# sndels/prosper

Measured on AMD Instinct MI355X. Metric: Mpaths/s, higher is better.
Workload: dtype f32; 1 GPU; S-cornell 1920x1080 8spp maxBounces 4; width=1920, height=1080, spp=8, max_bounces=4, triangles=38, bvh_nodes=7, parallelism=image stripes x1, pipeline=wavefront, 3 frames in flight (one launch chain each)

## Files before the change

include/prosper_pt/prosper_pt.h:

```cpp
#ifndef PROSPER_PT_H
#define PROSPER_PT_H

#include <stddef.h>
#include <stdint.h>

#include "shader_structs.h"

#ifdef __cplusplus
extern "C" {
#endif

#define PROSPER_PT_ABI_VERSION 4

enum
{
    PROSPER_PT_OK = 0,
    PROSPER_PT_ERR_INVALID_ARGUMENT = -1,
    PROSPER_PT_ERR_NO_DEVICE = -2,
    PROSPER_PT_ERR_HIP = -3,
    PROSPER_PT_ERR_NO_SCENE = -4,
    PROSPER_PT_ERR_SCENE = -5,
    PROSPER_PT_ERR_UNSUPPORTED = -6,
};

// ... 126 lines not shown
typedef struct prosper_pt_scene_stats
{
    uint64_t triangleCount;
    uint64_t nodeCount;
    uint32_t nodeBytes;
    uint32_t triangleBytes;
    uint32_t maxDepth;
    uint32_t variantFlags;
    uint64_t deviceBytes;
    double buildSeconds;
    double uploadSeconds;
    double bvhBuildSeconds;
    double textureSeconds;
    uint64_t alphaTriangleCount;
    uint64_t alphaBoundBytes;
} prosper_pt_scene_stats;
enum
{
    PROSPER_PT_VARIANT_LDS_SCENE = 1u << 0,
    PROSPER_PT_VARIANT_LDS_TABLES = 1u << 1,
    PROSPER_PT_VARIANT_BATCHED_TEXTURES = 1u << 2,
    PROSPER_PT_VARIANT_TEXTURE_PACKS = 1u << 3,
    PROSPER_PT_VARIANT_RAW_RECORDS = 1u << 4,
    PROSPER_PT_VARIANT_STACK_SHIFT = 8,
};

enum
{
    PROSPER_PT_RENDER_COUNT_WORK = 1u << 0,
    PROSPER_PT_RENDER_PIPELINED = 1u << 1,
};

typedef struct prosper_pt_debug_options
{
    uint32_t struct_size;
    int32_t batchedTextures;
    int32_t widePacks;
    int32_t alphaCellShift;
    uint32_t noTexturePacks;
    uint32_t noAlphaBounds;
    uint32_t noUploadRefit;
    uint32_t flatBvh;
    float sahTraversalCost;
    float boxPad;
    uint32_t leafSize;
    uint32_t buildThreads;
    uint32_t topEntries;
    int32_t nodeOrder;
    int32_t childOrder;
    uint32_t buildTiming;
    uint32_t segments;
    uint32_t segmentLength;
    uint32_t chains;
    uint32_t ldsStackEntries;
    uint32_t noLdsScene;
    uint32_t noLdsTables;
    uint32_t traceDeadPaths;
    int32_t bandedBatches;
    float rebuildCostRatio;
    uint32_t alwaysRebuild;
    uint32_t failNextUpdate;
    uint32_t poolVariant;
    uint32_t rawRecords;
    uint32_t tileOrder;
    uint32_t hipGraph;
    uint32_t pipelinedChains;
    uint32_t mergeLimit;
} prosper_pt_debug_options;

const char *prosper_pt_last_error(void);
uint32_t prosper_pt_abi_version(void);
uint32_t prosper_pt_has_experiments(void);
void prosper_pt_debug_options_default(prosper_pt_debug_options *out);
int prosper_pt_set_debug_options(prosper_pt_ctx *ctx, const prosper_pt_debug_options *options);
int prosper_pt_get_debug_options(prosper_pt_ctx *ctx, prosper_pt_debug_options *out);

int prosper_pt_create(const prosper_pt_device_desc *desc, prosper_pt_ctx **out_ctx);
void prosper_pt_destroy(prosper_pt_ctx *ctx);

int prosper_pt_upload_scene(prosper_pt_ctx *ctx, const prosper_pt_scene_view *scene);
int prosper_pt_update_lights(
    prosper_pt_ctx *ctx, const prosper_DirectionalLightParameters *directionalLight,
    const prosper_PointLightsBuffer *pointLights, const prosper_SpotLightsBuffer *spotLights);
int prosper_pt_update_transforms(prosper_pt_ctx *ctx, const prosper_ModelInstanceTransforms *transforms, uint32_t count);
enum
{
    PROSPER_PT_UPDATE_NOW = 1u << 0,
};
int prosper_pt_update_transforms_async(
    prosper_pt_ctx *ctx, const prosper_ModelInstanceTransforms *transforms, uint32_t count, uint32_t flags, void *stream);
// ... 228 lines not shown
```

prosper_amd/csrc/prosper_pt.cpp:

```cpp
#include "../../include/prosper_pt/prosper_pt.h"

#include <hip/hip_runtime.h>

#include <algorithm>
#include <chrono>
#include <future>
#include <memory>
#include <cmath>
#include <cstdlib>
#include <cstdio>
#include <cstring>
#include <exception>
#include <stdexcept>
#include <string>
#include <vector>

#include "bvh_build.hpp"
#include "pt_context.hpp"
#include "pt_geometry.hpp"
#include "pt_kernels.hpp"
#include "pt_materials.hpp"
#include "pt_pass_support.hpp"
#include "pt_scene.hpp"
#include "pt_tiling.hpp"
// ... 67 lines not shown
    if (e == hipSuccess && fill >= 0) e = hipMemset(buf.ptr, fill, allocBytes);
    if (e != hipSuccess)
    {
        if (buf.ptr) (void)hipFree(buf.ptr);
        buf.ptr = nullptr;
        return fail(PROSPER_PT_ERR_HIP, std::string("growing a device buffer: ") + hipGetErrorString(e));
    }
    buf.bytes = bytes;
    return PROSPER_PT_OK;
}

}

namespace
{

WavefrontOptions wavefront_options(const prosper_pt_ctx *ctx)
{
    const prosper_pt_debug_options &d = ctx->debug;
    WavefrontOptions o;
    o.ldsStackEntries = d.ldsStackEntries;
    o.noLdsScene = d.noLdsScene != 0;
    o.noLdsTables = d.noLdsTables != 0;
    return o;
}

}

namespace
{

void free_scene(prosper_pt_ctx *ctx)
{
    discard_mesh_build(ctx);
    for (ppt::AccelState *old : ctx->retiredAccel) delete old;
    ctx->retiredAccel.clear();
    for (auto &a : ctx->sceneAllocations) (void)hipFree(a.ptr);
    ctx->sceneAllocations.clear();
    delete ctx->accel;
    ctx->accel = nullptr;
    delete ctx->lights;
    ctx->lights = nullptr;
    delete ctx->materialState;
    ctx->materialState = nullptr;
    delete ctx->geometry;
    ctx->geometry = nullptr;
// ... 443 lines not shown
    if (o.chains > kMaxChains) return fail(PROSPER_PT_ERR_INVALID_ARGUMENT, "debug options: at most three launch chains");
    if (o.leafSize > 8u || o.alphaCellShift > 15 || o.nodeOrder > 2)
        return fail(PROSPER_PT_ERR_INVALID_ARGUMENT, "debug options: a value is out of range");
    if (!(o.sahTraversalCost >= 0.0f) || !(o.boxPad >= 0.0f) || !(o.rebuildCostRatio >= 0.0f))
        return fail(PROSPER_PT_ERR_INVALID_ARGUMENT, "debug options: a coefficient is negative or NaN");
    return PROSPER_PT_OK;
}

struct DebugField
{
    const char *name;
    size_t offset;
    char kind;
};
#define PPT_FIELD(member, kind) {#member, offsetof(prosper_pt_debug_options, member), kind}
const DebugField kDebugFields[] = {
    PPT_FIELD(batchedTextures, 'i'), PPT_FIELD(widePacks, 'i'), PPT_FIELD(alphaCellShift, 'i'), PPT_FIELD(noTexturePacks, 'u'),
    PPT_FIELD(noAlphaBounds, 'u'), PPT_FIELD(noUploadRefit, 'u'), PPT_FIELD(flatBvh, 'u'), PPT_FIELD(sahTraversalCost, 'f'),
    PPT_FIELD(boxPad, 'f'), PPT_FIELD(leafSize, 'u'), PPT_FIELD(buildThreads, 'u'), PPT_FIELD(topEntries, 'u'),
    PPT_FIELD(nodeOrder, 'i'), PPT_FIELD(childOrder, 'i'), PPT_FIELD(buildTiming, 'u'), PPT_FIELD(segments, 'u'),
    PPT_FIELD(segmentLength, 'u'), PPT_FIELD(chains, 'u'), PPT_FIELD(ldsStackEntries, 'u'), PPT_FIELD(noLdsScene, 'u'),
    PPT_FIELD(noLdsTables, 'u'), PPT_FIELD(traceDeadPaths, 'u'), PPT_FIELD(bandedBatches, 'i'), PPT_FIELD(rebuildCostRatio, 'f'), PPT_FIELD(alwaysRebuild, 'u'),
    PPT_FIELD(failNextUpdate, 'u'), PPT_FIELD(poolVariant, 'u'), PPT_FIELD(rawRecords, 'u'), PPT_FIELD(tileOrder, 'u'),
    PPT_FIELD(hipGraph, 'u'), PPT_FIELD(pipelinedChains, 'u'), PPT_FIELD(mergeLimit, 'u'),
};
#undef PPT_FIELD

bool parse_debug_options(const char *text, prosper_pt_debug_options *out, std::string *err)
{
    std::string rest = text ? text : "";
    while (!rest.empty())
    {
        const size_t comma = rest.find(',');
        const std::string item = rest.substr(0, comma);
        rest = comma == std::string::npos ? std::string() : rest.substr(comma + 1);
        if (item.empty()) continue;
        const size_t eq = item.find('=');
        const std::string name = item.substr(0, eq), value = eq == std::string::npos ? std::string("1") : item.substr(eq + 1);
        const DebugField *field = nullptr;
        for (const DebugField &f : kDebugFields)
            if (name == f.name) field = &f;
        if (!field)
        {
            *err = "debug options: unknown option '" + name + "'";
            return false;
        }
        char *end = nullptr;
// ... 598 lines not shown
    if (!ctx->haveScene || !ctx->accel) return fail(PROSPER_PT_ERR_NO_SCENE, "no scene uploaded");
    const size_t bytes = (size_t)ctx->accel->nodeCount * sizeof(BvhNode);
    if (byte_size < bytes) return fail(PROSPER_PT_ERR_INVALID_ARGUMENT, "prosper_pt_debug_read_nodes: destination too small");
    PPT_HIP(hipSetDevice(ctx->device));
    {
        const int frc = flush_pending_update(ctx, nullptr);
        if (frc != PROSPER_PT_OK) return frc;
    }
    PPT_HIP(hipDeviceSynchronize());
    PPT_HIP(hipMemcpy(out, ctx->accel->dNodes, bytes, hipMemcpyDeviceToHost));
    return PROSPER_PT_OK;
}

int prosper_pt_get_scene_stats(prosper_pt_ctx *ctx, prosper_pt_scene_stats *out)
{
    if (!ctx || !out) return fail(PROSPER_PT_ERR_INVALID_ARGUMENT, "prosper_pt_get_scene_stats: null argument");
    if (!ctx->haveScene) return fail(PROSPER_PT_ERR_NO_SCENE, "no scene uploaded");
    *out = ctx->stats;
    const WavefrontPlan plan = wavefront_plan(
        ctx->stats.maxDepth, (uint32_t)ctx->stats.nodeCount, (uint32_t)ctx->stats.triangleCount, ctx->scene, wavefront_options(ctx));
    const uint32_t ldsEntries = plan.ldsStackEntries;
    out->variantFlags =
        (plan.sceneInLds ? PROSPER_PT_VARIANT_LDS_SCENE : 0u) | (plan.tablesInLds ? PROSPER_PT_VARIANT_LDS_TABLES : 0u) |
        (ctx->scene.batchedTextures ? PROSPER_PT_VARIANT_BATCHED_TEXTURES : 0u) |
        (ctx->packedMaterials ? PROSPER_PT_VARIANT_TEXTURE_PACKS : 0u) |
        (ldsEntries << PROSPER_PT_VARIANT_STACK_SHIFT);
    return PROSPER_PT_OK;
}

int prosper_pt_set_output_buffer(prosper_pt_ctx *ctx, void *device_rgba32f, size_t byte_size)
{
    if (!ctx) return fail(PROSPER_PT_ERR_INVALID_ARGUMENT, "prosper_pt_set_output_buffer: null context");
    if (device_rgba32f && (reinterpret_cast<uintptr_t>(device_rgba32f) & 15u))
        return fail(PROSPER_PT_ERR_INVALID_ARGUMENT, "output buffer must be 16-byte aligned");
    ctx->externalHdr = device_rgba32f;
    ctx->externalHdrBytes = device_rgba32f ? byte_size : 0;
    return PROSPER_PT_OK;
}

int prosper_pt_render_frames(
    prosper_pt_ctx *ctx, const prosper_ReferencePC *pc, const prosper_CameraUniforms *camera, uint32_t width,
    uint32_t height, const prosper_pt_tile_desc *tile, uint32_t frame_count, uint32_t render_flags, void *stream)
{
    if (!ctx || !pc || !camera) return fail(PROSPER_PT_ERR_INVALID_ARGUMENT, "prosper_pt_render: null argument");
    if (!ctx->haveScene) return fail(PROSPER_PT_ERR_NO_SCENE, "prosper_pt_render called before prosper_pt_upload_scene");
    if (ctx->meshBuild)
// ... 395 lines not shown
```

prosper_amd/csrc/pt_device.hpp:

```cpp
#pragma once

#include "pt_math.hpp"
#include "pt_scene.hpp"

namespace ppt
{

#define PPT_D __device__ __forceinline__

constexpr uint32_t kMissIndex = 0xFFFFFFFFu;

struct LaneCounters
{
    uint32_t closestRays, shadowRays, nodeVisits, triangleTests, closestHits, anyHitCalls, lightSamples,
        spotLightSamples, skyLookups, shortIndexHits, paths, pixelsWritten, historyReads, shortIndexTriangleTests,
        nodePhaseSteps, trianglePhaseSteps, anyHitTexelFetches;
};


PPT_D uint32_t pcg(uint32_t v)
{
    const uint32_t state = v * 747796405u + 2891336453u;
    const uint32_t word = ((state >> ((state >> 28) + 4u)) ^ state) * 277803737u;
    return (word >> 22) ^ word;
// ... 874 lines not shown
    ray.tMax = kInf;
    return ray;
}

PPT_D float offset_component(float p, float n)
{
    const int32_t ofI = f2i(256.0f * n);
    const uint32_t moved = f2u(p) + (uint32_t)((p < 0.0f) ? -ofI : ofI);
    return fabs_(p) < (1.0f / 32.0f) ? __builtin_fmaf(1.0f / 65536.0f, n, p) : u2f(moved);
}
PPT_D f3 offset_ray(f3 p, f3 n)
{
    return f3{offset_component(p.x, n.x), offset_component(p.y, n.y), offset_component(p.z, n.z)};
}


PPT_D float safe_rcp_dir(float d)
{
    return 1.0f / (fabs_(d) < 1e-30f ? (d < 0.0f ? -1e-30f : 1e-30f) : d);
}

constexpr float kGuardPad = 1.52587890625e-05f;
constexpr float kGuardTol = 1.000003814697265625f;
PPT_D bool box_guard(f3 o, f3 invd, f3 v0, f3 v1, f3 v2, float tt)
{
    const float lox = fminf(fminf(v0.x, v1.x), v2.x), hix = fmaxf(fmaxf(v0.x, v1.x), v2.x);
    const float loy = fminf(fminf(v0.y, v1.y), v2.y), hiy = fmaxf(fmaxf(v0.y, v1.y), v2.y);
    const float loz = fminf(fminf(v0.z, v1.z), v2.z), hiz = fmaxf(fmaxf(v0.z, v1.z), v2.z);
    const float mx = fmaxf(fabs_(lox), fabs_(hix));
    const float my = fmaxf(fabs_(loy), fabs_(hiy));
    const float mz = fmaxf(fabs_(loz), fabs_(hiz));
    const float pad = fmaxf(fmaxf(mx, my), mz) * kGuardPad;
    const float ax = ((lox - pad) - o.x) * invd.x, bx = ((hix + pad) - o.x) * invd.x;
    const float ay = ((loy - pad) - o.y) * invd.y, by = ((hiy + pad) - o.y) * invd.y;
    const float az = ((loz - pad) - o.z) * invd.z, bz = ((hiz + pad) - o.z) * invd.z;
    const float tn = fmaxf(fmaxf(fminf(ax, bx), fminf(ay, by)), fminf(az, bz));
    const float tf = fminf(fminf(fmaxf(ax, bx), fmaxf(ay, by)), fmaxf(az, bz));
    return tn <= tt * kGuardTol && tt <= tf * kGuardTol;
}

struct EdgeFunctions
{
    float U, V, W, det;
    bool pass;
};
PPT_D EdgeFunctions edge_functions(f3 o, f3 d, f3 v0, f3 v1, f3 v2)
{
    const f3 A = v0 - o;
    const f3 B = v1 - o;
    const f3 C = v2 - o;
    EdgeFunctions e;
    e.U = dot(d, cross(C, B));
    e.V = dot(d, cross(A, C));
    e.W = dot(d, cross(B, A));
    e.det = (e.U + e.V) + e.W;
    const bool mixed = (e.U < 0.0f || e.V < 0.0f || e.W < 0.0f) && (e.U > 0.0f || e.V > 0.0f || e.W > 0.0f);
    e.pass = !mixed && e.det != 0.0f;
    return e;
}
PPT_D bool finish_triangle(
    const EdgeFunctions &e, f3 o, f3 d, f3 invd, f3 v0, f3 v1, f3 v2, float tMin, float tMax, float &t, float &bu, float &bv)
{
    const float inv = 1.0f / e.det;
    const float tt =
        __builtin_fmaf(e.W, dot(v2 - o, d), __builtin_fmaf(e.V, dot(v1 - o, d), e.U * dot(v0 - o, d))) * inv;
    if (!(tt > tMin && tt < tMax)) return false;
    if (!box_guard(o, invd, v0, v1, v2, tt)) return false;
    t = tt;
    bu = e.V * inv;
    bv = e.W * inv;
    return true;
}
PPT_D bool intersect_triangle(
    f3 o, f3 d, f3 invd, f3 v0, f3 v1, f3 v2, float tMin, float tMax, float &t, float &bu, float &bv)
{
    const EdgeFunctions e = edge_functions(o, d, v0, v1, v2);
    if (!e.pass) return false;
    return finish_triangle(e, o, d, invd, v0, v1, v2, tMin, tMax, t, bu, bv);
}

struct Hit
{
    uint32_t drawInstance;
    uint32_t primitive;
    f2 bary;
    float t;
};

struct AlphaFootprint
{
    global_u32_ptr texels;
    uint32_t o00, o10, o01, o11;
    float a, b;
    float factorA, cutoff, u;
// ... 321 lines not shown
    }
};
constexpr uint32_t kLdsNodeStrideHalf = 5;
struct LdsGeomHalf
{
    const float4 *nodes;
    const float4 *triangles;
    PPT_D NodeData node(int32_t i) const
    {
        const uint4 *np = reinterpret_cast<const uint4 *>(nodes + (uint32_t)i * kLdsNodeStrideHalf);
        return NodeData{np[0], np[1], np[2], np[3], np[4]};
    }
    template <bool SORTED>
    PPT_D void test_node(int32_t i, f3 o, const RaySlabs &rs, float tMin, float tMax, float e[4], int32_t ref[4]) const
    {
        intersect_node4<SORTED>(node(i), o, rs, tMin, tMax, e, ref);
    }
    PPT_D TriangleData tri(uint32_t i) const
    {
        const float4 *tp = triangles + i * 3u;
        return TriangleData{tp[0], tp[1], tp[2]};
    }
};
constexpr uint32_t kLdsSceneFloat4s = 768;

PPT_D bool descend_any(const float e[4], const int32_t ref[4], const TraversalStack &stack, int32_t &sp, int32_t &node)
{
    bool found = false;
    if (stack.ldsOnly || (uint32_t)sp + 3u <= stack.cap)
    {
#pragma unroll
        for (int k = 0; k < 4; ++k)
            if (e[k] < kInf)
            {
                if (found)
                    stack.lds[(uint32_t)(sp++) * stack.ldsStride] = ref[k];
                else
                {
                    node = ref[k];
                    found = true;
                }
            }
        return found;
    }
#pragma unroll
    for (int k = 0; k < 4; ++k)
        if (e[k] < kInf)
        {
            if (found)
                stack.push(sp, ref[k]);
            else
            {
                node = ref[k];
                found = true;
            }
        }
    return found;
}

template <bool ANY, bool COUNT, class Geom>
PPT_D bool trace_in(
    const Geom &g, const DeviceScene &s, f3 o, f3 d, float tMin, float tMaxIn, uint32_t seed, const TraversalStack &stack,
    Hit &hit, LaneCounters &cnt)
{
    hit.drawInstance = kMissIndex;
    hit.primitive = kMissIndex;
    hit.bary = f2{0.0f, 0.0f};
    hit.t = tMaxIn;
    const f3 invd = f3{safe_rcp_dir(d.x), safe_rcp_dir(d.y), safe_rcp_dir(d.z)};
    const RaySlabs rs = make_ray_slabs(invd);

    int32_t sp = 0;
    int32_t node = 0;
    bool alive = true;
    while (alive)
    {
        while (alive && node >= 0)
        {
            if constexpr (COUNT) cnt.nodeVisits++;
            float e[4];
            int32_t ref[4];
            bool entered;
            if constexpr (ANY)
            {
                g.template test_node<false>(node, o, rs, tMin, hit.t, e, ref);
                entered = descend_any(e, ref, stack, sp, node);
            }
            else
            {
                g.template test_node<true>(node, o, rs, tMin, hit.t, e, ref);
                stack.push_hit_children(sp, e, ref);
                entered = e[0] < kInf;
                if (entered) node = ref[0];
            }
            if (entered)
                ;
            else if (sp == 0)
                alive = false;
            else
                node = stack.pop(sp);
        }
        if (!alive) break;
        {
            const uint32_t ref = (uint32_t)~node;
            const uint32_t first = ref >> 3;
            const uint32_t count = (ref & 7u) + 1u;
            for (uint32_t i = 0; i < count; ++i)
            {
                const TriangleData td = g.tri(first + i);
                const float4 a = td.a, b = td.b, c = td.c;
                if constexpr (COUNT)
                {
                    cnt.triangleTests++;
                    cnt.shortIndexTriangleTests += (__builtin_bit_cast(uint32_t, c.w) & kTriFlagShortIndices) ? 1u : 0u;
                }
                float t, bu, bv;
                if (!intersect_triangle(
                        o, d, invd, f3{a.x, a.y, a.z}, f3{b.x, b.y, b.z}, f3{c.x, c.y, c.z}, tMin, tMaxIn, t, bu, bv))
                    continue;
                const uint32_t di = __builtin_bit_cast(uint32_t, a.w);
                const uint32_t prim = __builtin_bit_cast(uint32_t, b.w);
                const uint32_t flags = __builtin_bit_cast(uint32_t, c.w);
                if (!ANY && hit.drawInstance != kMissIndex)
                {
                    if (t > hit.t) continue;
                    if (t == hit.t && !(di < hit.drawInstance || (di == hit.drawInstance && prim < hit.primitive)))
                        continue;
                }
                if (!(flags & kTriFlagOpaque) && !any_hit_record<COUNT>(s, flags >> kTriAlphaShift, f2{bu, bv}, seed, cnt))
                    continue;
                hit.drawInstance = di;
                hit.primitive = prim;
                hit.bary = f2{bu, bv};
                hit.t = t;
                if (ANY) return true;
            }
        }
        if (sp == 0) break;
        node = stack.pop(sp);
    }
    return hit.drawInstance != kMissIndex;
}

template <bool ANY, bool COUNT>
PPT_D bool trace(
    const DeviceScene &s, f3 o, f3 d, float tMin, float tMaxIn, uint32_t seed, const TraversalStack &stack, Hit &hit,
    LaneCounters &cnt)
{
    return trace_in<ANY, COUNT>(GlobalGeom{s.nodes, s.triangles}, s, o, d, tMin, tMaxIn, seed, stack, hit, cnt);
}


PPT_D f3 mapped_normal(f3 tsn, f3 normal, f3 tangent, float sgn)
{
    const f3 vB = cross(normal, tangent) * sgn;
    return normalize(((tangent * tsn.x) + (vB * tsn.y)) + (normal * tsn.z));
}

template <bool COUNT, bool BATCHED_TEXTURES = false>
PPT_D Surface evaluate_surface(const DeviceScene &s, f3 rayDir, const Hit &hit, LaneCounters &cnt)
{
    const prosper_DrawInstance inst = s.drawInstances[hit.drawInstance];
    const uint32_t record = s.triangleOffsets[hit.drawInstance] + hit.primitive;
    Vertex v0, v1, v2;
    const float4 *rec = reinterpret_cast<const float4 *>(s.shadeTriangles + record);
    const float4 q0 = rec[0], q1 = rec[1], q2 = rec[2], q3 = rec[3], q4 = rec[4], q5 = rec[5], q6 = rec[6], q7 = rec[7];
// ... 142 lines not shown
```

prosper_amd/csrc/pt_kernels.hpp:

```cpp
#pragma once

#include <hip/hip_runtime.h>

#include "pt_scene.hpp"

namespace ppt
{

enum : uint32_t
{
    kStageGenerate = 0,
    kStageShade = 1,
    kStageTrace = 2,
    kStageAccumulate = 3,
    kStageCount = 4,
};

struct LaunchTimer
{
    hipEvent_t *events = nullptr;
    uint32_t *stage = nullptr;
    uint32_t count = 0;
    uint32_t capacity = 0;
    void mark(uint32_t st, hipStream_t stream)
// ... 30 lines not shown
uint32_t wavefront_grid_blocks(const WavefrontBuffers &w);
void launch_render_megakernel(
    const DeviceScene &s, const RenderParams &p, float4 *hdr, unsigned long long *counters, int32_t *stackOverflow,
    bool countWork, hipStream_t stream);
constexpr uint32_t kMaxChains = 3;
struct WavefrontChains
{
    uint32_t count = 1;
    bool detached = false;
    hipEvent_t after = nullptr;
    hipEvent_t scene = nullptr;
    hipEvent_t lights = nullptr;
    hipEvent_t materials = nullptr;
    hipStream_t streams[kMaxChains] = {};
    hipEvent_t fork = nullptr;
    hipEvent_t join[kMaxChains] = {};
    LaunchTimer *timers[kMaxChains] = {};
};
struct WavefrontPlan
{
    uint32_t ldsStackEntries;
    uint32_t overflowEntries;
    bool sceneInLds;
    bool tablesInLds;
    uint32_t scratchDwordsPerBlock;
};
struct WavefrontOptions
{
    uint32_t ldsStackEntries = 0;
    bool noLdsScene = false, noLdsTables = false;
};
WavefrontPlan wavefront_plan(
    uint32_t stackBound, uint32_t nodeCount, uint32_t triCount, const DeviceScene &s, const WavefrontOptions &opt);
void launch_render_wavefront(
    const DeviceScene &s, const RenderParams &p, float4 *hdr, unsigned long long *counters, const WavefrontBuffers &w,
    const WavefrontPlan &plan, int32_t *scratch, uint32_t nodeCount, uint32_t triCount, bool countWork, LaunchTimer *timer,
    const WavefrontChains &chains, hipStream_t stream);
uint32_t wavefront_lds_stack_entries(uint32_t stackBound, uint32_t forced);
bool wavefront_shade_tables_in_lds(const DeviceScene &s, bool disabled);
bool wavefront_scene_in_lds(uint32_t ldsStackEntries, uint32_t stackBound, uint32_t nodeCount, uint32_t triCount, bool disabled);
void launch_blit_rgba16f(const float4 *in, void *out, uint32_t count, hipStream_t stream);
constexpr uint32_t kMaxRanks = 64;
struct TileLayout
{
    uint32_t width, height, stripeWidth, ranks;
    uint32_t localWidth[kMaxRanks];
    uint64_t tileOffset[kMaxRanks];
};
void launch_deinterleave_tiles(const float4 *tiles, const TileLayout &layout, float4 *full, hipStream_t stream);
void launch_decode_bc7(
    const void *blocks, uint32_t width, uint32_t height, uint32_t tilesPerRow, void *tiled, hipStream_t stream);
void launch_retile_rgba8(const void *linear, uint32_t width, uint32_t height, uint32_t tilesPerRow, void *tiled, hipStream_t stream);
void launch_patch_alpha_records(AlphaTriangle *records, uint32_t count, const AlphaMaterial *table, uint32_t materialCount, hipStream_t stream);
// ... 8 lines not shown
```

prosper_amd/csrc/pt_wavefront.hip:

```cpp
#include "pt_kernels.hpp"

#include "pt_device.hpp"
#include "pt_render_common.hpp"
#include "pt_trace_stream.hpp"

#define PPT_SHADE_WPE 4
#ifndef PPT_GEN_WPE
#define PPT_GEN_WPE 5
#endif
#ifndef PPT_TRACE_WPE
#define PPT_TRACE_WPE(stack) 5
#endif

namespace ppt
{

namespace
{

constexpr uint32_t kSlotMask = 0x0FFFFFFFu;

struct SegmentId
{
    uint32_t seg;
// ... 211 lines not shown
    float *lf = reinterpret_cast<float *>(lds);
    for (uint32_t i = threadIdx.x; i < nodeCount * (kLdsNodeStride * 4u); i += blockDim.x)
    {
        const uint32_t n = i / (kLdsNodeStride * 4u), k = i - n * (kLdsNodeStride * 4u);
        const uint32_t q = k >> 2, c = k & 3u;
        float v = 0.0f;
        if (q == 0u)
            v = c < 3u ? gn[n].origin[c] : 0.0f;
        else if (q >= 1u && q <= 3u)
            v = half_to_float(gn[n].lo[q - 1u][c]);
        else if (q == 4u)
            v = __builtin_bit_cast(float, gn[n].child[c]);
        else if (q <= 7u)
            v = half_to_float(gn[n].hi[q - 5u][c]);
        lf[i] = v;
    }
    float4 *lt = lds + nodeCount * kLdsNodeStride;
    const float4 *gt = reinterpret_cast<const float4 *>(s.triangles);
    for (uint32_t i = threadIdx.x; i < triCount * 3u; i += blockDim.x) lt[i] = gt[i];
    __syncthreads();
    return LdsGeom{lds, lt};
}

}


template <bool COUNT, int STACK, bool LDS_SCENE>
__global__ __launch_bounds__(256, PPT_GEN_WPE) void wf_generate_extend(
    DeviceScene s, RenderParams p, WavefrontBuffers w, uint32_t nodeCount, uint32_t triCount,
    int32_t *__restrict__ stackOverflow, unsigned long long *__restrict__ counters)
{
    __shared__ int32_t ldsStack[STACK * 256];
    __shared__ float4 ldsScene[LDS_SCENE ? kLdsSceneFloat4s : 1];
    LdsGeomHalf lg = {};
    if constexpr (LDS_SCENE) lg = stage_scene_in_lds_half(s, ldsScene, nodeCount, triCount);
    const GlobalGeom gg{s.nodes, s.triangles};
    const SegmentId id = my_segment(w);
    if (!id.valid) return;
    const uint32_t lane = lane_id();
    const TraversalStack stack{(lds_int32 *)ldsStack + (threadIdx.x >> 6) * (STACK * 64u) + lane,
                               stackOverflow + blockIdx.x * 256u + threadIdx.x, (uint32_t)STACK, gridDim.x * 256u, 64u, LDS_SCENE};
    const bool traceRays = p.pc.maxBounces > 0;

    LaneCounters cnt = {};
    uint32_t nHit = 0;
    if (!traceRays)
    {
        for (uint32_t k = lane; k < w.segLen; k += 64u)
        {
            const SlotPixel sp = decode_slot(w, p, id.base + k);
            if (sp.valid)
            {
                if constexpr (COUNT) cnt.paths++;
                w.color[id.base + k] = make_float4(0.0f, 0.0f, 0.0f, 0.0f);
            }
        }
    }
    else
// ... 48 lines not shown
            {
                sst(&w.hit[id.base + pos], make_uint4(hit.drawInstance, hit.primitive, asu(hit.bary.x), asu(hit.bary.y)));
                sst(&w.hitIdx[id.base + pos], k);
            }
            nHit += total;
        };
        uint32_t dealStride = w.nSeg, dealFirst = id.seg, tileBase = 0u, tileCount = w.pixelsPadded >> 6;
        if (w.bandSegments != 0u)
        {
            const uint32_t band = id.seg / w.bandSegments;
            const uint32_t firstSeg = band * w.bandSegments;
            dealStride = w.nSeg - firstSeg < w.bandSegments ? w.nSeg - firstSeg : w.bandSegments;
            dealFirst = id.seg - firstSeg;
            tileBase = w.bandTile[band];
            tileCount = w.bandTile[band + 1u] - tileBase;
        }
        for (uint32_t k0 = 0; k0 < w.segLen; k0 += 64u)
        {
            const uint32_t k = k0 + lane;
            bl = batch_lane(w, p, (k0 >> 6) * dealStride + dealFirst, lane, tileBase, tileCount);
            const StreamRay r = fetch(k);
            Hit hit;
            bool found;
            if constexpr (LDS_SCENE)
                found = trace_in<false, COUNT>(lg, s, r.o, r.d, r.tMin, r.tMax, r.seed, stack, hit, cnt);
            else
                found = trace_in<false, COUNT>(gg, s, r.o, r.d, r.tMin, r.tMax, r.seed, stack, hit, cnt);
            commit(true, k, found, hit, r.d);
        }
    }
    if (lane == 0) w.segHits[id.seg] = nHit;
    flush_counters<COUNT>(cnt, counters);
}


template <bool COUNT, class Geom>
__device__ __forceinline__ uint32_t extend_segment(
    const Geom &g, const DeviceScene &s, const RenderParams &p, const WavefrontBuffers &w, const SegmentId &id, uint32_t n,
    uint32_t bounce, uint32_t cur, const TraversalStack &stack, LaneCounters &cnt)
{
    const float4 *__restrict__ rayA = w.rayA[cur];
    const float4 *__restrict__ rayB = w.rayB[cur];
    uint32_t nHit = 0;
    auto fetch = [&](uint32_t k) {
        const float4 a = sld(&rayA[id.base + k]);
        const float4 b = sld(&rayB[id.base + k]);
        if constexpr (COUNT) cnt.closestRays++;
// ... 295 lines not shown
    }
    flush_counters<COUNT>(cnt, counters);
}


template <bool COUNT, int STACK, bool LDS_SCENE>
static void enqueue_wavefront(
    const DeviceScene &s, const RenderParams &p, unsigned long long *counters, const WavefrontBuffers &w,
    const WavefrontPlan &plan, uint32_t nodeCount, uint32_t triCount, int32_t *stackOverflow, LaunchTimer *timer,
    hipStream_t stream)
{
    unsigned long long *cGen = counters + kStageGenerate * kCounterCount, *cShade = counters + kStageShade * kCounterCount,
                       *cTrace = counters + kStageTrace * kCounterCount;
    auto mark = [&](uint32_t st) {
        if (timer) timer->mark(st, stream);
    };
    const dim3 grid(((w.groupCount + 7u) / 8u) * 8u), block(256);
    uint32_t bounces = p.pc.maxBounces < PROSPER_RT_MAX_BOUNCES ? p.pc.maxBounces : PROSPER_RT_MAX_BOUNCES;
    const bool debugDraw =
        p.pc.drawType != PROSPER_DRAW_TYPE_DEFAULT && p.pc.drawType != PROSPER_DRAW_TYPE_MESHLET_ID;
    if (debugDraw && bounces > 1) bounces = 1;

    mark(kStageGenerate);
    hipLaunchKernelGGL(
        (wf_generate_extend<COUNT, STACK, LDS_SCENE>), grid, block, 0, stream, s, p, w, nodeCount, triCount,
        stackOverflow, cGen);
    for (uint32_t b = 0; b < bounces; ++b)
    {
        const uint32_t cur = b & 1u;
        const uint32_t last = (b + 1u == bounces) ? 1u : 0u;
        mark(kStageShade);
        const int ldsTables = !plan.tablesInLds ? 0 : (shade_table_bytes(s, true) <= kLdsTableBytes ? 1 : 2);
        auto shade = [&](auto kernel) { hipLaunchKernelGGL(kernel, grid, block, 0, stream, s, p, w, b, cur, last, cShade); };
        if (s.batchedTextures)
            ldsTables == 1 ? shade(wf_shade<COUNT, 1, true>) : (ldsTables == 2 ? shade(wf_shade<COUNT, 2, true>) : shade(wf_shade<COUNT, 0, true>));
        else
            ldsTables == 1 ? shade(wf_shade<COUNT, 1, false>) : (ldsTables == 2 ? shade(wf_shade<COUNT, 2, false>) : shade(wf_shade<COUNT, 0, false>));
        if (!debugDraw)
        {
            mark(kStageTrace);
            hipLaunchKernelGGL(
                (wf_trace<COUNT, STACK, LDS_SCENE>), grid, block, 0, stream, s, p, w, b, cur ^ 1u, last ? 0u : 1u,
                nodeCount, triCount, stackOverflow, cTrace);
        }
    }
}

uint32_t wavefront_grid_blocks(const WavefrontBuffers &w)
{
// ... 3 lines not shown

uint32_t wavefront_lds_stack_entries(uint32_t stackBound, uint32_t forced)
{
    if (forced == 16u || forced == 24u || forced == 32u) return forced;
    return stackBound <= 16u ? 16u : 24u;
}

bool wavefront_shade_tables_in_lds(const DeviceScene &s, bool disabled)
{
    return shade_table_bytes(s, false) <= kLdsTableBytes && !disabled;
}
bool wavefront_scene_in_lds(uint32_t ldsStackEntries, uint32_t stackBound, uint32_t nodeCount, uint32_t triCount, bool disabled)
{
    return ldsStackEntries == 16u && stackBound <= 16u && nodeCount * kLdsNodeStride + triCount * 3u <= kLdsSceneFloat4s && !disabled;
}

WavefrontPlan wavefront_plan(
    uint32_t stackBound, uint32_t nodeCount, uint32_t triCount, const DeviceScene &s, const WavefrontOptions &opt)
{
    WavefrontPlan plan = {};
    plan.ldsStackEntries = wavefront_lds_stack_entries(stackBound, opt.ldsStackEntries);
    plan.overflowEntries = stackBound > plan.ldsStackEntries ? stackBound - plan.ldsStackEntries : 0u;
    plan.sceneInLds = wavefront_scene_in_lds(plan.ldsStackEntries, stackBound, nodeCount, triCount, opt.noLdsScene);
    plan.tablesInLds = wavefront_shade_tables_in_lds(s, opt.noLdsTables);
    plan.scratchDwordsPerBlock = plan.overflowEntries * 256u;
    return plan;
}

template <bool COUNT>
static void enqueue_for_stack(
    const DeviceScene &s, const RenderParams &p, unsigned long long *counters, const WavefrontBuffers &w,
    const WavefrontPlan &plan, int32_t *stackOverflow, uint32_t nodeCount, uint32_t triCount, LaunchTimer *timer,
    hipStream_t stream)
{
    if (plan.sceneInLds)
        enqueue_wavefront<COUNT, 16, true>(s, p, counters, w, plan, nodeCount, triCount, stackOverflow, timer, stream);
    else if (plan.ldsStackEntries == 16u)
        enqueue_wavefront<COUNT, 16, false>(s, p, counters, w, plan, nodeCount, triCount, stackOverflow, timer, stream);
    else if (plan.ldsStackEntries == 24u)
        enqueue_wavefront<COUNT, 24, false>(s, p, counters, w, plan, nodeCount, triCount, stackOverflow, timer, stream);
    else
        enqueue_wavefront<COUNT, 32, false>(s, p, counters, w, plan, nodeCount, triCount, stackOverflow, timer, stream);
}

void launch_render_wavefront(
    const DeviceScene &s, const RenderParams &p, float4 *hdr, unsigned long long *counters, const WavefrontBuffers &w,
// ... 49 lines not shown
```

prosper_amd/structs.py:

```python
import ctypes as C

import numpy as np


class Vec4(C.Structure):
    _fields_ = [("x", C.c_float), ("y", C.c_float), ("z", C.c_float), ("w", C.c_float)]


class Mat4(C.Structure):
    _fields_ = [("col", Vec4 * 4)]


class Mat3x4(C.Structure):
    _fields_ = [("col", Vec4 * 3)]


class ReferencePC(C.Structure):

    _fields_ = [
        ("drawType", C.c_uint32),
        ("flags", C.c_uint32),
        ("frameIndex", C.c_uint32),
        ("apertureDiameter", C.c_float),
        ("focusDistance", C.c_float),
# ... 232 lines not shown
        ("textureSeconds", C.c_double),
        ("alphaTriangleCount", C.c_uint64),
        ("alphaBoundBytes", C.c_uint64),
    ]


class HierarchyState(C.Structure):
    _fields_ = [("refits", C.c_uint32), ("rebuilds", C.c_uint32), ("costRatio", C.c_float), ("builtCost", C.c_float),
                ("nodeCount", C.c_uint32), ("levels", C.c_uint32), ("meshUpdates", C.c_uint32), ("geometryInstalls", C.c_uint32),
                ("geometryBuildRunning", C.c_uint32), ("reserved", C.c_uint32)]


class DebugOptions(C.Structure):

    _fields_ = [("struct_size", C.c_uint32),
                ("batchedTextures", C.c_int32), ("widePacks", C.c_int32), ("alphaCellShift", C.c_int32),
                ("noTexturePacks", C.c_uint32), ("noAlphaBounds", C.c_uint32), ("noUploadRefit", C.c_uint32), ("flatBvh", C.c_uint32),
                ("sahTraversalCost", C.c_float), ("boxPad", C.c_float), ("leafSize", C.c_uint32), ("buildThreads", C.c_uint32),
                ("topEntries", C.c_uint32), ("nodeOrder", C.c_int32), ("childOrder", C.c_int32), ("buildTiming", C.c_uint32),
                ("segments", C.c_uint32), ("segmentLength", C.c_uint32), ("chains", C.c_uint32), ("ldsStackEntries", C.c_uint32),
                ("noLdsScene", C.c_uint32), ("noLdsTables", C.c_uint32), ("traceDeadPaths", C.c_uint32), ("bandedBatches", C.c_int32),
                ("rebuildCostRatio", C.c_float), ("alwaysRebuild", C.c_uint32), ("failNextUpdate", C.c_uint32),
                ("poolVariant", C.c_uint32), ("rawRecords", C.c_uint32), ("tileOrder", C.c_uint32), ("hipGraph", C.c_uint32),
                ("pipelinedChains", C.c_uint32), ("mergeLimit", C.c_uint32)]


class CommInfo(C.Structure):
    _fields_ = [("ranks", C.c_uint32), ("rank", C.c_uint32), ("device", C.c_int32), ("gathers", C.c_uint32),
                ("lastGatherMs", C.c_float), ("reserved", C.c_uint32)]


class MeshUpdate(C.Structure):
    _fields_ = [("meshIndex", C.c_uint32), ("reserved", C.c_uint32), ("metadata", GeometryMetadata), ("info", MeshInfo),
                ("bytes", C.c_void_p), ("byteOffset", C.c_uint64), ("byteCount", C.c_uint64), ("bufferByteSize", C.c_uint64)]


MAX_GEOMETRY_BUFFERS = 100
GATHER_IN_STREAM = 1
UPDATE_NOW = 1
VARIANT_LDS_SCENE = 1
VARIANT_LDS_TABLES = 2
VARIANT_BATCHED_TEXTURES = 4
VARIANT_TEXTURE_PACKS = 8
VARIANT_RAW_RECORDS = 16
VARIANT_STACK_SHIFT = 8


def as_numpy(struct_array, dtype=np.uint8):
    return np.frombuffer(struct_array, dtype=dtype)


class RestirTracePC(C.Structure):
    _fields_ = [("drawType", C.c_uint32), ("frameIndex", C.c_uint32), ("flags", C.c_uint32)]


class RestirInputs(C.Structure):
    _fields_ = [("albedoRoughness", C.c_void_p), ("normalMetallic", C.c_void_p), ("nonLinearDepth", C.c_void_p),
                ("reservoirs", C.c_void_p), ("onDevice", C.c_uint32), ("reserved", C.c_uint32)]


RESTIR_INITIAL = 0
RESTIR_SPATIAL = 1
RESTIR_SPATIAL_REUSE = 1

RESTIR_TRACE_GBUFFER = 1 << 1
RESTIR_JITTER_GBUFFER = 1 << 2
GBUFFER_JITTER = 1 << 0
# ... 29 lines not shown
```

Before: 8870 Mpaths/s.

## Stage eye-relative BVH and precomputed triangle edge crosses in LDS for camera rays

For the generate/extend kernel, the scene is staged in LDS already translated to the camera eye, with node planes stored as full floats in both near and far orders and the triangle edge cross products and guard planes precomputed. Camera rays then skip the origin subtraction and the cross products in each node and triangle test, using only dot products with the ray direction. This trades a larger LDS footprint (7 float4 per node and per triangle) and a heavier per-block staging step for cheaper primary-ray traversal. It is enabled only when the scene fits and depth of field is off.

```diff
diff --git a/include/prosper_pt/prosper_pt.h b/include/prosper_pt/prosper_pt.h
--- a/include/prosper_pt/prosper_pt.h
+++ b/include/prosper_pt/prosper_pt.h
@@ -172,6 +172,7 @@
     PROSPER_PT_VARIANT_BATCHED_TEXTURES = 1u << 2,
     PROSPER_PT_VARIANT_TEXTURE_PACKS = 1u << 3,
     PROSPER_PT_VARIANT_RAW_RECORDS = 1u << 4,
+    PROSPER_PT_VARIANT_EYE_GEOMETRY = 1u << 5,
     PROSPER_PT_VARIANT_STACK_SHIFT = 8,
 };
 
@@ -216,6 +217,7 @@
     uint32_t hipGraph;
     uint32_t pipelinedChains;
     uint32_t mergeLimit;
+    uint32_t noEyeGeometry;
 } prosper_pt_debug_options;
 
 const char *prosper_pt_last_error(void);
diff --git a/prosper_amd/csrc/prosper_pt.cpp b/prosper_amd/csrc/prosper_pt.cpp
--- a/prosper_amd/csrc/prosper_pt.cpp
+++ b/prosper_amd/csrc/prosper_pt.cpp
@@ -113,6 +113,7 @@
     o.ldsStackEntries = d.ldsStackEntries;
     o.noLdsScene = d.noLdsScene != 0;
     o.noLdsTables = d.noLdsTables != 0;
+    o.noEyeGeometry = d.noEyeGeometry != 0;
     return o;
 }
 
@@ -602,7 +603,7 @@
     PPT_FIELD(segmentLength, 'u'), PPT_FIELD(chains, 'u'), PPT_FIELD(ldsStackEntries, 'u'), PPT_FIELD(noLdsScene, 'u'),
     PPT_FIELD(noLdsTables, 'u'), PPT_FIELD(traceDeadPaths, 'u'), PPT_FIELD(bandedBatches, 'i'), PPT_FIELD(rebuildCostRatio, 'f'), PPT_FIELD(alwaysRebuild, 'u'),
     PPT_FIELD(failNextUpdate, 'u'), PPT_FIELD(poolVariant, 'u'), PPT_FIELD(rawRecords, 'u'), PPT_FIELD(tileOrder, 'u'),
-    PPT_FIELD(hipGraph, 'u'), PPT_FIELD(pipelinedChains, 'u'), PPT_FIELD(mergeLimit, 'u'),
+    PPT_FIELD(hipGraph, 'u'), PPT_FIELD(pipelinedChains, 'u'), PPT_FIELD(mergeLimit, 'u'), PPT_FIELD(noEyeGeometry, 'u'),
 };
 #undef PPT_FIELD
 
@@ -1247,6 +1248,7 @@
     const uint32_t ldsEntries = plan.ldsStackEntries;
     out->variantFlags =
         (plan.sceneInLds ? PROSPER_PT_VARIANT_LDS_SCENE : 0u) | (plan.tablesInLds ? PROSPER_PT_VARIANT_LDS_TABLES : 0u) |
+        (plan.eyeGeometry ? PROSPER_PT_VARIANT_EYE_GEOMETRY : 0u) |
         (ctx->scene.batchedTextures ? PROSPER_PT_VARIANT_BATCHED_TEXTURES : 0u) |
         (ctx->packedMaterials ? PROSPER_PT_VARIANT_TEXTURE_PACKS : 0u) |
         (ldsEntries << PROSPER_PT_VARIANT_STACK_SHIFT);
diff --git a/prosper_amd/csrc/pt_device.hpp b/prosper_amd/csrc/pt_device.hpp
--- a/prosper_amd/csrc/pt_device.hpp
+++ b/prosper_amd/csrc/pt_device.hpp
@@ -920,7 +920,11 @@
 
 constexpr float kGuardPad = 1.52587890625e-05f;
 constexpr float kGuardTol = 1.000003814697265625f;
-PPT_D bool box_guard(f3 o, f3 invd, f3 v0, f3 v1, f3 v2, float tt)
+struct GuardPlanes
+{
+    f3 lo, hi;
+};
+PPT_D GuardPlanes guard_planes(f3 o, f3 v0, f3 v1, f3 v2)
 {
     const float lox = fminf(fminf(v0.x, v1.x), v2.x), hix = fmaxf(fmaxf(v0.x, v1.x), v2.x);
     const float loy = fminf(fminf(v0.y, v1.y), v2.y), hiy = fmaxf(fmaxf(v0.y, v1.y), v2.y);
@@ -929,45 +933,63 @@
     const float my = fmaxf(fabs_(loy), fabs_(hiy));
     const float mz = fmaxf(fabs_(loz), fabs_(hiz));
     const float pad = fmaxf(fmaxf(mx, my), mz) * kGuardPad;
-    const float ax = ((lox - pad) - o.x) * invd.x, bx = ((hix + pad) - o.x) * invd.x;
-    const float ay = ((loy - pad) - o.y) * invd.y, by = ((hiy + pad) - o.y) * invd.y;
-    const float az = ((loz - pad) - o.z) * invd.z, bz = ((hiz + pad) - o.z) * invd.z;
+    return GuardPlanes{f3{(lox - pad) - o.x, (loy - pad) - o.y, (loz - pad) - o.z}, f3{(hix + pad) - o.x, (hiy + pad) - o.y, (hiz + pad) - o.z}};
+}
+PPT_D bool guard_test(const GuardPlanes &g, f3 invd, float tt)
+{
+    const float ax = g.lo.x * invd.x, bx = g.hi.x * invd.x;
+    const float ay = g.lo.y * invd.y, by = g.hi.y * invd.y;
+    const float az = g.lo.z * invd.z, bz = g.hi.z * invd.z;
     const float tn = fmaxf(fmaxf(fminf(ax, bx), fminf(ay, by)), fminf(az, bz));
     const float tf = fminf(fminf(fmaxf(ax, bx), fmaxf(ay, by)), fmaxf(az, bz));
     return tn <= tt * kGuardTol && tt <= tf * kGuardTol;
 }
+PPT_D bool box_guard(f3 o, f3 invd, f3 v0, f3 v1, f3 v2, float tt)
+{
+    return guard_test(guard_planes(o, v0, v1, v2), invd, tt);
+}
 
 struct EdgeFunctions
 {
     float U, V, W, det;
     bool pass;
 };
-PPT_D EdgeFunctions edge_functions(f3 o, f3 d, f3 v0, f3 v1, f3 v2)
-{
-    const f3 A = v0 - o;
-    const f3 B = v1 - o;
-    const f3 C = v2 - o;
+PPT_D EdgeFunctions edge_functions_of(f3 d, f3 cCB, f3 cAC, f3 cBA)
+{
     EdgeFunctions e;
-    e.U = dot(d, cross(C, B));
-    e.V = dot(d, cross(A, C));
-    e.W = dot(d, cross(B, A));
+    e.U = dot(d, cCB);
+    e.V = dot(d, cAC);
+    e.W = dot(d, cBA);
     e.det = (e.U + e.V) + e.W;
     const bool mixed = (e.U < 0.0f || e.V < 0.0f || e.W < 0.0f) && (e.U > 0.0f || e.V > 0.0f || e.W > 0.0f);
     e.pass = !mixed && e.det != 0.0f;
     return e;
 }
-PPT_D bool finish_triangle(
-    const EdgeFunctions &e, f3 o, f3 d, f3 invd, f3 v0, f3 v1, f3 v2, float tMin, float tMax, float &t, float &bu, float &bv)
+PPT_D EdgeFunctions edge_functions(f3 o, f3 d, f3 v0, f3 v1, f3 v2)
+{
+    const f3 A = v0 - o;
+    const f3 B = v1 - o;
+    const f3 C = v2 - o;
+    return edge_functions_of(d, cross(C, B), cross(A, C), cross(B, A));
+}
+template <class GuardFn>
+PPT_D bool finish_triangle_rel(
+    const EdgeFunctions &e, f3 d, f3 invd, f3 A, f3 B, f3 C, const GuardFn &guard, float tMin, float tMax, float &t, float &bu,
+    float &bv)
 {
     const float inv = 1.0f / e.det;
-    const float tt =
-        __builtin_fmaf(e.W, dot(v2 - o, d), __builtin_fmaf(e.V, dot(v1 - o, d), e.U * dot(v0 - o, d))) * inv;
+    const float tt = __builtin_fmaf(e.W, dot(C, d), __builtin_fmaf(e.V, dot(B, d), e.U * dot(A, d))) * inv;
     if (!(tt > tMin && tt < tMax)) return false;
-    if (!box_guard(o, invd, v0, v1, v2, tt)) return false;
+    if (!guard_test(guard(), invd, tt)) return false;
     t = tt;
     bu = e.V * inv;
     bv = e.W * inv;
     return true;
+}
+PPT_D bool finish_triangle(
+    const EdgeFunctions &e, f3 o, f3 d, f3 invd, f3 v0, f3 v1, f3 v2, float tMin, float tMax, float &t, float &bu, float &bv)
+{
+    return finish_triangle_rel(e, d, invd, v0 - o, v1 - o, v2 - o, [&]() { return guard_planes(o, v0, v1, v2); }, tMin, tMax, t, bu, bv);
 }
 PPT_D bool intersect_triangle(
     f3 o, f3 d, f3 invd, f3 v0, f3 v1, f3 v2, float tMin, float tMax, float &t, float &bu, float &bv)
@@ -1335,6 +1357,56 @@
         return TriangleData{tp[0], tp[1], tp[2]};
     }
 };
+constexpr uint32_t kLdsNodeStrideEye = 7;
+constexpr uint32_t kLdsTriStrideEye = 7;
+struct LdsGeomEye
+{
+    const float4 *nodes;
+    const float4 *triangles;
+    template <bool SORTED>
+    PPT_D void test_node(int32_t i, const RaySlabs &rs, float tMin, float tMax, float e[4], int32_t ref[4]) const
+    {
+        typedef float f4n __attribute__((ext_vector_type(4)));
+        typedef uint32_t u4n __attribute__((ext_vector_type(4)));
+        typedef __attribute__((address_space(3))) const f4n *lds_f4;
+        typedef __attribute__((address_space(3))) const u4n *lds_u4;
+        const uint32_t base = (uint32_t)(uintptr_t)(__attribute__((address_space(3))) const void *)nodes + (uint32_t)i * (kLdsNodeStrideEye * 16u);
+        const uint32_t sx = (__builtin_bit_cast(uint32_t, rs.invd.x) >> 25) & 64u;
+        const uint32_t sy = (__builtin_bit_cast(uint32_t, rs.invd.y) >> 25) & 64u;
+        const uint32_t sz = (__builtin_bit_cast(uint32_t, rs.invd.z) >> 25) & 64u;
+        const f4n nx = *(lds_f4)(uintptr_t)(base + sx), fx = *(lds_f4)(uintptr_t)(base + 64u - sx);
+        const f4n ny = *(lds_f4)(uintptr_t)(base + 16u + sy), fy = *(lds_f4)(uintptr_t)(base + 80u - sy);
+        const f4n nz = *(lds_f4)(uintptr_t)(base + 32u + sz), fz = *(lds_f4)(uintptr_t)(base + 96u - sz);
+        const u4n ch = *(lds_u4)(uintptr_t)(base + 48u);
+        const uint4 children = make_uint4(ch.x, ch.y, ch.z, ch.w);
+        const v2f tnx01 = v2f{nx.x, nx.y} * rs.invd.x, tnx23 = v2f{nx.z, nx.w} * rs.invd.x;
+        const v2f tny01 = v2f{ny.x, ny.y} * rs.invd.y, tny23 = v2f{ny.z, ny.w} * rs.invd.y;
+        const v2f tnz01 = v2f{nz.x, nz.y} * rs.invd.z, tnz23 = v2f{nz.z, nz.w} * rs.invd.z;
+        const v2f tfx01 = v2f{fx.x, fx.y} * rs.invdK.x, tfx23 = v2f{fx.z, fx.w} * rs.invdK.x;
+        const v2f tfy01 = v2f{fy.x, fy.y} * rs.invdK.y, tfy23 = v2f{fy.z, fy.w} * rs.invdK.y;
+        const v2f tfz01 = v2f{fz.x, fz.y} * rs.invdK.z, tfz23 = v2f{fz.z, fz.w} * rs.invdK.z;
+        finish_node4<SORTED>(tnx01, tnx23, tny01, tny23, tnz01, tnz23, tfx01, tfx23, tfy01, tfy23, tfz01, tfz23, children, tMin, tMax, e, ref);
+    }
+    PPT_D TriangleData tri(uint32_t i) const
+    {
+        const float4 *tp = triangles + i * kLdsTriStrideEye;
+        return TriangleData{tp[0], tp[1], tp[2]};
+    }
+    PPT_D bool finish(uint32_t i, const EdgeFunctions &e, f3 d, f3 invd, float tMin, float tMax, float &t, float &bu, float &bv) const
+    {
+        const float4 *tp = triangles + i * kLdsTriStrideEye;
+        const float4 a = tp[3], b = tp[4], c = tp[5];
+        const auto guard = [&]() {
+            const float4 h = tp[6];
+            return GuardPlanes{f3{a.w, b.w, c.w}, f3{h.x, h.y, h.z}};
+        };
+        return finish_triangle_rel(e, d, invd, f3{a.x, a.y, a.z}, f3{b.x, b.y, b.z}, f3{c.x, c.y, c.z}, guard, tMin, tMax, t, bu, bv);
+    }
+};
+template <class Geom>
+inline constexpr bool kEyeRelativeGeom = false;
+template <>
+inline constexpr bool kEyeRelativeGeom<LdsGeomEye> = true;
 constexpr uint32_t kLdsSceneFloat4s = 768;
 
 PPT_D bool descend_any(const float e[4], const int32_t ref[4], const TraversalStack &stack, int32_t &sp, int32_t &node)
@@ -1376,6 +1448,7 @@
     const Geom &g, const DeviceScene &s, f3 o, f3 d, float tMin, float tMaxIn, uint32_t seed, const TraversalStack &stack,
     Hit &hit, LaneCounters &cnt)
 {
+    static_assert(!(ANY && kEyeRelativeGeom<Geom>), "eye-relative geometry serves closest-hit camera rays only");
     hit.drawInstance = kMissIndex;
     hit.primitive = kMissIndex;
     hit.bary = f2{0.0f, 0.0f};
@@ -1401,7 +1474,10 @@
             }
             else
             {
-                g.template test_node<true>(node, o, rs, tMin, hit.t, e, ref);
+                if constexpr (kEyeRelativeGeom<Geom>)
+                    g.template test_node<true>(node, rs, tMin, hit.t, e, ref);
+                else
+                    g.template test_node<true>(node, o, rs, tMin, hit.t, e, ref);
                 stack.push_hit_children(sp, e, ref);
                 entered = e[0] < kInf;
                 if (entered) node = ref[0];
@@ -1428,8 +1504,14 @@
                     cnt.shortIndexTriangleTests += (__builtin_bit_cast(uint32_t, c.w) & kTriFlagShortIndices) ? 1u : 0u;
                 }
                 float t, bu, bv;
-                if (!intersect_triangle(
-                        o, d, invd, f3{a.x, a.y, a.z}, f3{b.x, b.y, b.z}, f3{c.x, c.y, c.z}, tMin, tMaxIn, t, bu, bv))
+                if constexpr (kEyeRelativeGeom<Geom>)
+                {
+                    const EdgeFunctions ef = edge_functions_of(d, f3{a.x, a.y, a.z}, f3{b.x, b.y, b.z}, f3{c.x, c.y, c.z});
+                    if (!ef.pass) continue;
+                    if (!g.finish(first + i, ef, d, invd, tMin, tMaxIn, t, bu, bv)) continue;
+                }
+                else if (!intersect_triangle(
+                             o, d, invd, f3{a.x, a.y, a.z}, f3{b.x, b.y, b.z}, f3{c.x, c.y, c.z}, tMin, tMaxIn, t, bu, bv))
                     continue;
                 const uint32_t di = __builtin_bit_cast(uint32_t, a.w);
                 const uint32_t prim = __builtin_bit_cast(uint32_t, b.w);
@@ -1455,6 +1537,14 @@
     return hit.drawInstance != kMissIndex;
 }
 
+template <bool COUNT>
+PPT_D bool trace_in(
+    const LdsGeomEye &g, const DeviceScene &s, f3 d, float tMin, float tMaxIn, uint32_t seed, const TraversalStack &stack,
+    Hit &hit, LaneCounters &cnt)
+{
+    return trace_in<false, COUNT>(g, s, f3{0.0f, 0.0f, 0.0f}, d, tMin, tMaxIn, seed, stack, hit, cnt);
+}
+
 template <bool ANY, bool COUNT>
 PPT_D bool trace(
     const DeviceScene &s, f3 o, f3 d, float tMin, float tMaxIn, uint32_t seed, const TraversalStack &stack, Hit &hit,
diff --git a/prosper_amd/csrc/pt_kernels.hpp b/prosper_amd/csrc/pt_kernels.hpp
--- a/prosper_amd/csrc/pt_kernels.hpp
+++ b/prosper_amd/csrc/pt_kernels.hpp
@@ -76,13 +76,14 @@
     uint32_t ldsStackEntries;
     uint32_t overflowEntries;
     bool sceneInLds;
+    bool eyeGeometry;
     bool tablesInLds;
     uint32_t scratchDwordsPerBlock;
 };
 struct WavefrontOptions
 {
     uint32_t ldsStackEntries = 0;
-    bool noLdsScene = false, noLdsTables = false;
+    bool noLdsScene = false, noLdsTables = false, noEyeGeometry = false;
 };
 WavefrontPlan wavefront_plan(
     uint32_t stackBound, uint32_t nodeCount, uint32_t triCount, const DeviceScene &s, const WavefrontOptions &opt);
diff --git a/prosper_amd/csrc/pt_wavefront.hip b/prosper_amd/csrc/pt_wavefront.hip
--- a/prosper_amd/csrc/pt_wavefront.hip
+++ b/prosper_amd/csrc/pt_wavefront.hip
@@ -257,18 +257,66 @@
     return LdsGeom{lds, lt};
 }
 
-}
-
-
-template <bool COUNT, int STACK, bool LDS_SCENE>
+__device__ __forceinline__ LdsGeomEye stage_scene_in_lds_eye(
+    const DeviceScene &s, f3 eye, float4 *lds, uint32_t nodeCount, uint32_t triCount)
+{
+    const BvhNode *gn = s.nodes;
+    float *lf = reinterpret_cast<float *>(lds);
+    for (uint32_t i = threadIdx.x; i < nodeCount * (kLdsNodeStrideEye * 4u); i += blockDim.x)
+    {
+        const uint32_t n = i / (kLdsNodeStrideEye * 4u), k = i - n * (kLdsNodeStrideEye * 4u);
+        const uint32_t q = k >> 2, c = k & 3u;
+        float v;
+        if (q == 3u)
+            v = __builtin_bit_cast(float, gn[n].child[c]);
+        else
+        {
+            const bool far = q > 3u;
+            const uint32_t a = far ? q - 4u : q;
+            const float oRel = (a == 0u ? eye.x : (a == 1u ? eye.y : eye.z)) - gn[n].origin[a];
+            v = half_to_float(far ? gn[n].hi[a][c] : gn[n].lo[a][c]) - oRel;
+        }
+        lf[i] = v;
+    }
+    float4 *lt = lds + nodeCount * kLdsNodeStrideEye;
+    const float4 *gt = reinterpret_cast<const float4 *>(s.triangles);
+    for (uint32_t i = threadIdx.x; i < triCount; i += blockDim.x)
+    {
+        const float4 a = gt[i * 3u], b = gt[i * 3u + 1u], c = gt[i * 3u + 2u];
+        const f3 v0 = xyz(a), v1 = xyz(b), v2 = xyz(c);
+        const f3 A = v0 - eye, B = v1 - eye, C = v2 - eye;
+        const f3 cCB = cross(C, B), cAC = cross(A, C), cBA = cross(B, A);
+        const GuardPlanes g = guard_planes(eye, v0, v1, v2);
+        float4 *out = lt + i * kLdsTriStrideEye;
+        out[0] = make_float4(cCB.x, cCB.y, cCB.z, a.w);
+        out[1] = make_float4(cAC.x, cAC.y, cAC.z, b.w);
+        out[2] = make_float4(cBA.x, cBA.y, cBA.z, c.w);
+        out[3] = make_float4(A.x, A.y, A.z, g.lo.x);
+        out[4] = make_float4(B.x, B.y, B.z, g.lo.y);
+        out[5] = make_float4(C.x, C.y, C.z, g.lo.z);
+        out[6] = make_float4(g.hi.x, g.hi.y, g.hi.z, 0.0f);
+    }
+    __syncthreads();
+    return LdsGeomEye{lds, lt};
+}
+
+}
+
+
+template <bool COUNT, int STACK, bool LDS_SCENE, bool EYE = false>
 __global__ __launch_bounds__(256, PPT_GEN_WPE) void wf_generate_extend(
     DeviceScene s, RenderParams p, WavefrontBuffers w, uint32_t nodeCount, uint32_t triCount,
     int32_t *__restrict__ stackOverflow, unsigned long long *__restrict__ counters)
 {
+    static_assert(!EYE || LDS_SCENE, "the eye-relative image lives in LDS");
     __shared__ int32_t ldsStack[STACK * 256];
     __shared__ float4 ldsScene[LDS_SCENE ? kLdsSceneFloat4s : 1];
     LdsGeomHalf lg = {};
-    if constexpr (LDS_SCENE) lg = stage_scene_in_lds_half(s, ldsScene, nodeCount, triCount);
+    LdsGeomEye le = {};
+    if constexpr (EYE)
+        le = stage_scene_in_lds_eye(s, f3{p.eye[0], p.eye[1], p.eye[2]}, ldsScene, nodeCount, triCount);
+    else if constexpr (LDS_SCENE)
+        lg = stage_scene_in_lds_half(s, ldsScene, nodeCount, triCount);
     const GlobalGeom gg{s.nodes, s.triangles};
     const SegmentId id = my_segment(w);
     if (!id.valid) return;
@@ -363,7 +411,9 @@
             const StreamRay r = fetch(k);
             Hit hit;
             bool found;
-            if constexpr (LDS_SCENE)
+            if constexpr (EYE)
+                found = trace_in<COUNT>(le, s, r.d, r.tMin, r.tMax, r.seed, stack, hit, cnt);
+            else if constexpr (LDS_SCENE)
                 found = trace_in<false, COUNT>(lg, s, r.o, r.d, r.tMin, r.tMax, r.seed, stack, hit, cnt);
             else
                 found = trace_in<false, COUNT>(gg, s, r.o, r.d, r.tMin, r.tMax, r.seed, stack, hit, cnt);
@@ -705,9 +755,16 @@
     if (debugDraw && bounces > 1) bounces = 1;
 
     mark(kStageGenerate);
-    hipLaunchKernelGGL(
-        (wf_generate_extend<COUNT, STACK, LDS_SCENE>), grid, block, 0, stream, s, p, w, nodeCount, triCount,
-        stackOverflow, cGen);
+    bool eye = false;
+    if constexpr (LDS_SCENE) eye = plan.eyeGeometry && !(p.pc.flags & PROSPER_PC_FLAG_DEPTH_OF_FIELD);
+    if (eye)
+        hipLaunchKernelGGL(
+            (wf_generate_extend<COUNT, STACK, LDS_SCENE, LDS_SCENE>), grid, block, 0, stream, s, p, w, nodeCount, triCount,
+            stackOverflow, cGen);
+    else
+        hipLaunchKernelGGL(
+            (wf_generate_extend<COUNT, STACK, LDS_SCENE>), grid, block, 0, stream, s, p, w, nodeCount, triCount,
+            stackOverflow, cGen);
     for (uint32_t b = 0; b < bounces; ++b)
     {
         const uint32_t cur = b & 1u;
@@ -757,6 +814,8 @@
     plan.ldsStackEntries = wavefront_lds_stack_entries(stackBound, opt.ldsStackEntries);
     plan.overflowEntries = stackBound > plan.ldsStackEntries ? stackBound - plan.ldsStackEntries : 0u;
     plan.sceneInLds = wavefront_scene_in_lds(plan.ldsStackEntries, stackBound, nodeCount, triCount, opt.noLdsScene);
+    plan.eyeGeometry = plan.sceneInLds && !opt.noEyeGeometry &&
+                       nodeCount * kLdsNodeStrideEye + triCount * kLdsTriStrideEye <= kLdsSceneFloat4s;
     plan.tablesInLds = wavefront_shade_tables_in_lds(s, opt.noLdsTables);
     plan.scratchDwordsPerBlock = plan.overflowEntries * 256u;
     return plan;
diff --git a/prosper_amd/structs.py b/prosper_amd/structs.py
--- a/prosper_amd/structs.py
+++ b/prosper_amd/structs.py
@@ -278,7 +278,8 @@
                 ("noLdsScene", C.c_uint32), ("noLdsTables", C.c_uint32), ("traceDeadPaths", C.c_uint32), ("bandedBatches", C.c_int32),
                 ("rebuildCostRatio", C.c_float), ("alwaysRebuild", C.c_uint32), ("failNextUpdate", C.c_uint32),
                 ("poolVariant", C.c_uint32), ("rawRecords", C.c_uint32), ("tileOrder", C.c_uint32), ("hipGraph", C.c_uint32),
-                ("pipelinedChains", C.c_uint32), ("mergeLimit", C.c_uint32)]
+                ("pipelinedChains", C.c_uint32), ("mergeLimit", C.c_uint32),
+                ("noEyeGeometry", C.c_uint32)]
 
 
 class CommInfo(C.Structure):
@@ -299,6 +300,7 @@
 VARIANT_BATCHED_TEXTURES = 4
 VARIANT_TEXTURE_PACKS = 8
 VARIANT_RAW_RECORDS = 16
+VARIANT_EYE_GEOMETRY = 32
 VARIANT_STACK_SHIFT = 8
 
 
```

Result: no change. 8949 Mpaths/s, median of 5 (+0.9%).
